# inferflow/inferflow

Measured on AMD Instinct MI355X. Metric: decode tokens/sec, Llama-2-7B Q4 batch=1 greedy (whole job), higher is better.
Workload: dtype i8 (Q8 activations x Q4_B32T1A weights, i32 dot, f32 scale, f16 I/O); 1 GPU; llama2_7b decode, Q4_B32T1A weights + F16 lm_head, F16 KV cache, batch 1 greedy, 16-token prompt, context 21..1851; parallelism=single, weights_bytes=4309647360

## Files before the change

include/inferflow_amd.h:

```cpp
#ifndef INFERFLOW_AMD_H_
#define INFERFLOW_AMD_H_

#include <stddef.h>
#include <stdint.h>

#ifdef __cplusplus
extern "C" {
#endif

typedef enum {
    IFA_F32 = 0, IFA_F16 = 1,
    IFA_Q8_B32T1 = 7, IFA_Q8_B32T2 = 8, IFA_Q6_B64T1 = 9, IFA_Q5_B64T1 = 10, IFA_Q5_B32T1 = 11,
    IFA_Q4_B16 = 12, IFA_Q4_B32T1A = 13, IFA_Q4_B32T1B = 14, IFA_Q4_B64T1 = 17, IFA_Q3H_B64T1 = 18,
    IFA_Q3_B32T1A = 19, IFA_Q3_B32T1B = 20, IFA_Q2_B32T1A = 21, IFA_Q2_B32T1B = 22
} ifa_dtype;

enum {
    IFA_OK = 0,
    IFA_ERR_ARG = -1,
    IFA_ERR_DTYPE = -2,
    IFA_ERR_HIP = -3,
    IFA_ERR_STATE = -4,
    IFA_ERR_NOMEM = -5
};
// ... 111 lines not shown
    IFA_T_EMBD = 0, IFA_T_OUT_NORM = 1, IFA_T_OUT_NORM_B = 2, IFA_T_LM_HEAD = 3,
    IFA_T_ATTN_NORM = 10, IFA_T_ATTN_NORM_B = 11, IFA_T_WQ = 12, IFA_T_WK = 13, IFA_T_WV = 14, IFA_T_WO = 15,
    IFA_T_FFN_NORM = 16, IFA_T_FFN_NORM_B = 17, IFA_T_W1 = 18, IFA_T_W2 = 19, IFA_T_W3 = 20, IFA_T_MOE_GATE = 21,
    IFA_T_WQ_B = 22, IFA_T_WK_B = 23, IFA_T_WV_B = 24, IFA_T_WO_B = 25, IFA_T_W1_B = 26, IFA_T_W2_B = 27, IFA_T_W3_B = 28,
    IFA_T_ATTN_POST_NORM = 29, IFA_T_ATTN_POST_NORM_B = 30, IFA_T_FFN_POST_NORM = 31, IFA_T_FFN_POST_NORM_B = 32
};

int ifa_model_create(const ifa_model_config *cfg, ifa_model **out);
int ifa_model_destroy(ifa_model *m);
int ifa_model_set_tensor(ifa_model *m, int layer, int tensor_id, int expert, int dtype,
                         const void *dev_src, size_t rows, size_t cols);
int ifa_model_set_tensor_f16(ifa_model *m, int layer, int tensor_id, int expert, int target_dtype,
                             const void *dev_src_f16, size_t rows, size_t cols);
int ifa_model_finalize(ifa_model *m);
int ifa_model_reset(ifa_model *m);
int ifa_model_kv_slots(ifa_model *m, int n_slots);
int ifa_model_select_kv(ifa_model *m, int slot);
int ifa_model_kv_copy(ifa_model *m, int src_slot, int dst_slot, int n_rows);
int ifa_model_set_option(ifa_model *m, const char *name, int value);
int ifa_model_set_excluded_tokens(ifa_model *m, const int *ids_host, int n);
int ifa_model_perf_stat(ifa_model *m, int *keys_out, float *ms_out, int cap, int *n_out, int clear);
int ifa_model_fused_supported(ifa_model *m, char *why, size_t why_len);
int ifa_model_forward(ifa_model *m, const int *tokens_host, int n_tokens, int prefix_len,
                      void *logits_out_dev, int *next_token_host);
int ifa_model_decode(ifa_model *m, int first_token, int start_pos, int n_steps,
                     int *out_tokens_host, float *elapsed_ms);
int ifa_model_decode_prepare(ifa_model *m, int start_pos, int n_steps);
int ifa_model_decode_batch(ifa_model *m, int n, const int *tokens_host, const int *positions_host, const int *kv_slots_host,
                           int *next_tokens_host, void *logits_out_dev);
int ifa_model_decode_draft(ifa_model *m, int n, const int *tokens_host, int pos0, int *next_tokens_host, void *logits_out_dev);
// ... 72 lines not shown
```

inferflow_amd/_capi.py:

```python
import ctypes as C
import os

_HERE = os.path.dirname(os.path.abspath(__file__))
_LIB_PATH = os.environ.get("IFA_LIB") or os.path.join(_HERE, "lib", "libinferflow_amd.so")
_lib = None


class IfaError(RuntimeError):
    def __init__(self, code, msg):
        super().__init__("inferflow_amd error %d: %s" % (code, msg))
        self.code = code


def library_path():
    return _LIB_PATH


def lib():
    global _lib
    if _lib is None:
        if not os.path.exists(_LIB_PATH):
            raise ImportError(
                "inferflow_amd: %s is missing -- run `python __graft_entry__.py build` "
                "(hipcc --offload-arch=gfx950); there is no CPU fallback" % _LIB_PATH)
# ... 81 lines not shown
    "ifa_add_by_row_index": (_i, [_vp, _vp, _sz, _sz, _vp, _vp, _vp]),
    "ifa_model_kv_slots": (_i, [_vp, _i]),
    "ifa_model_select_kv": (_i, [_vp, _i]),
    "ifa_model_kv_copy": (_i, [_vp, _i, _i, _i]),
    "ifa_model_decode_batch": (_i, [_vp, _i, _vp, _vp, _vp, _vp, _vp]),
    "ifa_model_decode_draft": (_i, [_vp, _i, _vp, _i, _vp, _vp]),
    "ifa_model_set_pool_excluded": (_i, [_vp, _vp, _i]),
    "ifa_model_decode_pool": (_i, [_vp, _i, _i, _i, _vp, _vp, _vp, _vp]),
    "ifa_model_decode_batch_pool": (_i, [_vp, _i, _vp, _vp, _vp, _vp, _i, _vp, _i, _vp, _vp, _vp]),
    "ifa_model_forward_pool": (_i, [_vp, _vp, _i, _i, _vp, _i, _vp, _vp, _vp, _vp]),
    "ifa_model_pool_lse": (_i, [_vp, _vp, _i, _vp]),
    "ifa_model_forward_score": (_i, [_vp, _vp, _i, _i, _vp, _vp, _vp, _vp]),
    "ifa_model_get_buffer": (_i, [_vp, C.c_char_p, _i, C.POINTER(_vp), C.POINTER(_sz)]),
    "ifa_model_stream": (_vp, [_vp]),
    "ifa_model_time_kernel": (_i, [_vp, _i, _i, _vp]),
    "ifa_model_set_stream": (_i, [_vp, _vp]),
    "ifa_model_tp_begin": (_i, [_vp, _i, _i]),
    "ifa_model_tp_begin_hidden": (_i, [_vp, _vp, _i]),
    "ifa_model_tp_hidden": (_i, [_vp, _vp]),
    "ifa_model_tp_attn": (_i, [_vp, _i, _vp]),
    "ifa_model_tp_post_attn": (_i, [_vp, _i, _vp]),
    "ifa_model_tp_ffn": (_i, [_vp, _i, _vp]),
    "ifa_model_tp_post_ffn": (_i, [_vp, _i, _vp]),
    "ifa_model_tp_logits": (_i, [_vp, _vp]),
    "ifa_model_tp_set_token": (_i, [_vp, _vp]),
    "ifa_comm_unique_id": (_i, [_vp]),
    "ifa_comm_init_rank": (_i, [_vp, _i, _i, _i, C.POINTER(_vp)]),
    "ifa_comm_init_all": (_i, [_vp, _i, C.POINTER(_vp)]),
    "ifa_comm_destroy": (_i, [_vp]),
    "ifa_comm_capturable": (_i, [_vp]),
# ... 93 lines not shown
```

inferflow_amd/csrc/ifa_decode_qkv_attn.h:

```cpp
#pragma once
#include "ifa_decode_kernels.h"
#include "ifa_decode_attn.h"

namespace ifa {

struct DecQkvAttnExtra {
    unsigned long long *gran;
    const unsigned *epoch;
    unsigned epoch_add;
    unsigned *err;
    int timeout_us;
    int gk;
    int unload;
};

#ifndef IFA_QA_EARLY_KV
#define IFA_QA_EARLY_KV 0
#endif
#ifndef IFA_QA_WARM_ROWS
#define IFA_QA_WARM_ROWS 1
#endif
constexpr int QA_THREADS = 512;

template <int DT, int NJ, int RW, int NORM, int HD, bool Q8, int PB, bool KT, int NP, bool UL = false>
__global__ void __launch_bounds__(QA_THREADS) k_dec_qkv_attn(const half_t *px, const half_t *pnw, const half_t *pnb, int pcols, int pgeo,
                                                             const uint8_t *pwq, const uint8_t *pwk, const uint8_t *pwv,
                                                             const DecGemvParams P, const DecAttnParams A, const DecQkvAttnExtra E)
{
    const int g_heads = pgeo & 0xFF, g_kvh = (pgeo >> 8) & 0xFF, g_gk = (pgeo >> 16) & 0xFFFF;
    const int g_nblk = pcols / block_capacity(DT);
    extern __shared__ __attribute__((aligned(16))) char smem[];
    const long long t_kernel = wall_clock64();
    static_assert(NORM == 0 || NORM == 1, "QKV prologue: quantiser with or without the RMS norm");
    static_assert(NP > 0 && NP * 64 < QA_THREADS, "wave-specialised prologue");
    constexpr int TH = QA_THREADS, PT = NP * 64;
    constexpr int MAXC = (NJ * 8 * block_capacity(DT) + PT - 1) / PT;
    XPre<NORM, MAXC, false, PT> pre;
    if (threadIdx.x < PT) pre.issue(px, pnw, pnb, pcols);
    const XLds L = xlds_carve(smem, pcols);
    const int lane = threadIdx.x & 63;
    const int wave = __builtin_amdgcn_readfirstlane(threadIdx.x >> 6);
    using Fmt = DecFmt<DT, NJ>;
    const size_t row_bytes = tiled_row_bytes(DT, (size_t)g_nblk);
    const int g = (int)blockIdx.x / g_gk, bg = (int)blockIdx.x - g * g_gk;
    const int group = g_heads / g_kvh;
    const int RG = (group + 2) * HD;
    const int per = g_gk / group;
    const bool attn_wg = bg % per == 0;
    const int head = g * group + bg / per;
    const int WGV = UL ? (g_gk - group) * (TH / 64) : g_gk * (TH / 64);
    const int lw = UL ? (bg - bg / per - 1) * (TH / 64) + wave : bg * (TH / 64) + wave;
    struct Row { const uint8_t *w; const half_t *b; half_t *y; int row, vrow; };
    auto locate = [&](int lr) {
        Row r;
        const int nq = group * HD;
        const bool isk = lr >= nq && lr < nq + HD, isv = lr >= nq + HD;
        r.row = isv ? g * HD + (lr - nq - HD) : (isk ? g * HD + (lr - nq) : g * nq + lr);
        r.w = isv ? P.W0[2] : (isk ? P.W0[1] : P.W0[0]);
        r.b = isv ? P.b0[2] : (isk ? P.b0[1] : P.b0[0]);
// ... 20 lines not shown
                if (i < i0 || i >= i1) continue;
                if (i > 0 && i * WGV + lw >= RG) continue;
                w[i].load(wrow(min(i * WGV + lw, RG - 1)), g_nblk, lane);
            }
        }
    };
    static_assert(NP == 4, "the prologue waves are the attention waves");
    const bool ul_head = UL && attn_wg;
    if (!ul_head && threadIdx.x == TH - 1) { L.part[130] = 0.0f; L.part[131] = 0.0f; }
    if (!ul_head && wave >= NP) load_rows(0, 1);
    const int pos = *(const __attribute__((address_space(4))) int *)(A.state + 1);
    const unsigned epoch = ((*(const __attribute__((address_space(4))) unsigned *)(E.epoch) + E.epoch_add) << 20) | ((unsigned)pos & 0xFFFFFu);
    DecAttnFusedIn F;
    F.gran = E.gran; F.epoch = epoch; F.pos = pos; F.err = E.err; F.timeout_ticks = (long long)E.timeout_us * 100;
    F.att_gran = nullptr;
    if constexpr (UL) {
        if (attn_wg) {
            if (wave >= 4) {
#if IFA_QA_WARM_ROWS
                if (pos >= PB) {
                    constexpr int SB = Q8 ? (HD / 32) * 34 : HD * 2;
                    const int kvh = head / group, kv_dim = g_kvh * HD;
                    const size_t rb = Q8 ? (size_t)(kv_dim / 32) * 34 : (size_t)kv_dim * 2;
                    const size_t ho = Q8 ? (size_t)((kvh * HD) / 32) * 34 : (size_t)kvh * HD * 2;
                    const int t = (int)threadIdx.x - 256;
                    const int off = min((t & 3) * 64, SB - 4) & ~1;
                    typedef uint32_t u32_a2 __attribute__((aligned(2)));
                    uint32_t acc = 0;
                    for (int j = PB + (t >> 2); j <= pos; j += 64) {
                        acc ^= *(const __attribute__((address_space(1))) u32_a2 *)(A.kcache + (size_t)j * rb + ho + off);
                        acc ^= *(const __attribute__((address_space(1))) u32_a2 *)(A.vcache + (size_t)j * rb + ho + off);
                    }
                    if (acc == 0x9E3779B9u && A.trace) A.trace[(size_t)A.heads * 8 + 7] = (long long)acc;
                }
#endif
                return;
            }
            DecAttnRegs<HD, Q8, PB, KT> RU;
            dec_attn_body<HD, Q8, false, PB, KT, true>(smem, nullptr, A.kcache, A.vcache, A.heads, A.kv_heads, A, head, F, RU);
            return;
        }
    }
    __syncthreads();
    DecAttnRegs<HD, Q8, PB, KT> R;
    if (wave >= NP) {
        load_rows(1, RW);
    } else {
        pre.finish(P.norm_w, P.norm_b, P.multi_base, P.eps, P.cols, L, P.xn_out, nullptr);
        load_rows(0, RW);
#if IFA_QA_EARLY_KV
        if (attn_wg) dec_attn_body<HD, Q8, false, PB, KT, true, 1>(smem, nullptr, A.kcache, A.vcache, A.heads, A.kv_heads, A, head, F, R);
#endif
    }
    lds_counter_wait(L.part + 131, NP);
    typename Fmt::X X;
    X.load(L.codes, L.scale, L.xsum, lane, g_nblk);
    {
        float a[RW];
#pragma unroll
        for (int i = 0; i < RW; i++) a[i] = w[i].dot(X);
#pragma unroll
        for (int i = 0; i < RW; i++) a[i] = wave_sum(a[i]);
        float a0 = 0.0f;
#pragma unroll
        for (int i = 0; i < RW; i++) { if (lane == i) a0 = a[i]; }
        const int lr = lane * WGV + lw;
        if (lane < RW && lr < RG) {
            const Row r = locate(lr);
            half_t y = dec_bias(a0, r.b, r.row);
            if (P.pre_scale != 0.0f) y = f2h(h2f(y) * P.pre_scale);
            r.y[r.row] = y;
            __hip_atomic_store(E.gran + r.vrow, ((unsigned long long)epoch << 32) | (unsigned long long)__builtin_bit_cast(uint16_t, y),
                               __ATOMIC_RELAXED, __HIP_MEMORY_SCOPE_AGENT);
        }
    }
    if (A.trace && threadIdx.x == 0) {
        A.trace[(size_t)(A.heads + (int)blockIdx.x) * 8 + 0] = t_kernel;
        A.trace[(size_t)(A.heads + (int)blockIdx.x) * 8 + 1] = wall_clock64();
    }
    if (attn_wg) {
        __syncthreads();
        if (wave >= 4) return;
        dec_attn_body<HD, Q8, false, PB, KT, true, IFA_QA_EARLY_KV ? 2 : 0>(smem, nullptr, A.kcache, A.vcache, A.heads, A.kv_heads, A, head, F, R);
        return;
    }
}

bool dec_qkv_attn_supported(int w_dtype, int cols, int heads, int kv_heads, int head_dim, int num_cus, int *gk_out, int *rw_out);
int dec_qkv_attn_launch(int w_dtype, int norm, bool kv_q8, int pb, bool kt, const DecGemvParams &P, const DecAttnParams &A, const DecQkvAttnExtra &E,
                        int max_ctx, hipStream_t s);
template <int DT>
int dec_qkv_attn_launch_dt(int norm, bool kv_q8, int pb, bool kt, int rw, const DecGemvParams &P, const DecAttnParams &A, const DecQkvAttnExtra &E,
                           int max_ctx, hipStream_t s);
// ... 3 lines not shown
```

inferflow_amd/csrc/ifa_dqkvattn_q4b32.hip:

```cpp
#include <algorithm>
#include "ifa_dqkvattn_impl.h"

namespace ifa {

extern template int dec_qkv_attn_launch_dt<Q3H_B64T1>(int, bool, int, bool, int, const DecGemvParams &, const DecAttnParams &, const DecQkvAttnExtra &, int, hipStream_t);
template int dec_qkv_attn_launch_dt<Q4_B32T1A>(int, bool, int, bool, int, const DecGemvParams &, const DecAttnParams &, const DecQkvAttnExtra &, int, hipStream_t);

bool dec_qkv_attn_supported(int w_dtype, int cols, int heads, int kv_heads, int head_dim, int num_cus, int *gk_out, int *rw_out)
{
    const bool q4 = w_dtype == Q4_B32T1A || w_dtype == Q4_B32T1B;
    if (!q4 && w_dtype != Q3H_B64T1) return false;
    if (head_dim != 128 || cols != 4096 || kv_heads < 1 || heads % kv_heads != 0) return false;
    if (num_cus < kv_heads || num_cus % kv_heads != 0) return false;
    const int gk = num_cus / kv_heads, group = heads / kv_heads;
    if (gk % group != 0) return false;
    const int rg = (group + 2) * head_dim, wv = gk * (QA_THREADS / 64);
    if (rg % wv != 0) return false;
    const int rw = rg / wv;
    if (rw != 6 && rw != 3) return false;
    if (gk_out) *gk_out = gk;
    if (rw_out) *rw_out = rw;
    return true;
}

// ... 3 lines not shown
    DecGemvParams P = P0;
    P.trace = nullptr;
    P.total_rows = P.rows[0] + P.rows[1] + P.rows[2];
    P.nblk = P.cols / block_capacity(w_dtype);
    int gk = 0, rw = 0;
    if (!dec_qkv_attn_supported(w_dtype, P.cols, A.heads, A.kv_heads, 128, A.kv_heads * E.gk, &gk, &rw) || gk != E.gk)
        return ifa_fail(IFA_ERR_ARG, "fused QKV + attention: unsupported shape");
    switch (w_dtype) {
    case Q4_B32T1A: case Q4_B32T1B: return dec_qkv_attn_launch_dt<Q4_B32T1A>(norm, kv_q8, pb, kt, rw, P, A, E, max_ctx, s);
    case Q3H_B64T1: return dec_qkv_attn_launch_dt<Q3H_B64T1>(norm, kv_q8, pb, kt, rw, P, A, E, max_ctx, s);
    default: return ifa_fail(IFA_ERR_DTYPE, "fused QKV + attention: dtype %d", w_dtype);
    }
}

}
```

inferflow_amd/csrc/ifa_engine.hip:

```cpp
#include "ifa_engine_state.h"

namespace ifae {

int perf_begin(ifa_model *m, int key)
{
    if (!m->opt_perf_stat) return -1;
    hipStreamCaptureStatus cs = hipStreamCaptureStatusNone;
    if (hipStreamIsCapturing(m->stream, &cs) != hipSuccess || cs != hipStreamCaptureStatusNone) { (void)hipGetLastError(); return -1; }
    auto take = [&]() -> hipEvent_t {
        if (!m->perf_pool.empty()) { hipEvent_t e = m->perf_pool.back(); m->perf_pool.pop_back(); return e; }
        hipEvent_t e = nullptr;
        if (hipEventCreate(&e) != hipSuccess) { (void)hipGetLastError(); return nullptr; }
        return e;
    };
    ifa_model::PerfSpanRec r; r.key = key; r.e0 = take(); r.e1 = take();
    if (!r.e0 || !r.e1) { if (r.e0) m->perf_pool.push_back(r.e0); if (r.e1) m->perf_pool.push_back(r.e1); return -1; }
    if (hipEventRecord(r.e0, m->stream) != hipSuccess) { (void)hipGetLastError(); m->perf_pool.push_back(r.e0); m->perf_pool.push_back(r.e1); return -1; }
    m->perf_spans.push_back(r);
    return (int)m->perf_spans.size() - 1;
}

void perf_end(ifa_model *m, int idx)
{
    if (idx < 0 || idx >= (int)m->perf_spans.size()) return;
// ... 6 lines not shown
    IFA_HIP_CHECK(hipStreamSynchronize(m->stream));
    for (auto &r : m->perf_spans) {
        float ms = 0.0f;
        if (hipEventElapsedTime(&ms, r.e0, r.e1) == hipSuccess) m->perf_map[r.key] += ms;
        else (void)hipGetLastError();
        m->perf_pool.push_back(r.e0); m->perf_pool.push_back(r.e1);
    }
    m->perf_spans.clear();
    return IFA_OK;
}

void drop_graphs(ifa_model *m)
{
    if (m->tp_graph_exec) { (void)hipGraphExecDestroy(m->tp_graph_exec); m->tp_graph_exec = nullptr; }
    if (m->tp_graph) { (void)hipGraphDestroy(m->tp_graph); m->tp_graph = nullptr; }
    if (m->graph_exec) { (void)hipGraphExecDestroy(m->graph_exec); m->graph_exec = nullptr; }
    if (m->graph) { (void)hipGraphDestroy(m->graph); m->graph = nullptr; }
    if (m->graph_exec_n) { (void)hipGraphExecDestroy(m->graph_exec_n); m->graph_exec_n = nullptr; }
    if (m->graph_n) { (void)hipGraphDestroy(m->graph_n); m->graph_n = nullptr; }
    for (auto &sl : m->slots) {
        if (sl.exec) { (void)hipGraphExecDestroy(sl.exec); sl.exec = nullptr; }
        if (sl.graph) { (void)hipGraphDestroy(sl.graph); sl.graph = nullptr; }
    }
    for (auto &kv : m->batch_graphs) if (kv.second) (void)hipGraphExecDestroy(kv.second);
    m->batch_graphs.clear();
    for (auto &kv : m->draft_graphs) if (kv.second) (void)hipGraphExecDestroy(kv.second);
    m->draft_graphs.clear();
}

void free_tensor(Tensor &t)
{
    if (t.data) (void)hipFree(t.data);
    if (t.tiled) (void)hipFree(t.tiled);
    if (t.mo) (void)hipFree(t.mo);
    if (t.x32) (void)hipFree(t.x32);
    if (t.q3hn) (void)hipFree(t.q3hn);
    t = Tensor();
}
// ... 430 lines not shown
    IFA_HIP_CHECK(hipStreamSynchronize(m->stream));
    return IFA_OK;
}

int ifa_model_select_kv(ifa_model *m, int slot)
{
    IFA_REQUIRE(m && m->finalized, "ifa_model_select_kv: model not finalized");
    if (m->slots.empty()) m->slots.resize(1);
    IFA_REQUIRE(slot >= 0 && slot < (int)m->slots.size(), "ifa_model_select_kv: slot %d of %zu", slot, m->slots.size());
    if (slot == m->cur_slot) return IFA_OK;
    if (m->tp_graph_exec) { (void)hipGraphExecDestroy(m->tp_graph_exec); m->tp_graph_exec = nullptr; }
    if (m->tp_graph) { (void)hipGraphDestroy(m->tp_graph); m->tp_graph = nullptr; }
    ifa_model::KvSlot &out = m->slots[(size_t)m->cur_slot], &in = m->slots[(size_t)slot];
    out.k.clear(); out.v.clear();
    for (Layer &L : m->layers) { out.k.push_back(L.kcache); out.v.push_back(L.vcache); }
    out.graph = m->graph; out.exec = m->graph_exec;
    if (m->graph_exec_n) { (void)hipGraphExecDestroy(m->graph_exec_n); m->graph_exec_n = nullptr; }
    if (m->graph_n) { (void)hipGraphDestroy(m->graph_n); m->graph_n = nullptr; }
    for (size_t l = 0; l < m->layers.size(); l++) { m->layers[l].kcache = in.k[l]; m->layers[l].vcache = in.v[l]; }
    m->graph = in.graph; m->graph_exec = in.exec;
    in.k.clear(); in.v.clear(); in.graph = nullptr; in.exec = nullptr;
    m->cur_slot = slot;
    return IFA_OK;
}

int ifa_model_set_option(ifa_model *m, const char *name, int value)
{
    IFA_REQUIRE(m && name, "ifa_model_set_option: null pointer");
    if (strcmp(name, "pool_lse") == 0) { m->opt_pool_lse = value != 0; return IFA_OK; }
    struct { const char *n; int *p; } opts[] = {
        {"fused", &m->opt_fused}, {"graph", &m->opt_graph}, {"rpw_qkv", &m->opt_rpw_qkv}, {"rpw_wo", &m->opt_rpw_wo},
        {"rpw_ffn", &m->opt_rpw_ffn}, {"rpw_w2", &m->opt_rpw_w2}, {"rpw_lm", &m->opt_rpw_lm}, {"trace", &m->opt_trace},
        {"bench_mode", &m->opt_bench_mode}, {"touch_stride", &m->opt_touch_stride}, {"attn_split_ctx", &m->opt_attn_split_ctx}, {"batch_graph", &m->opt_batch_graph}, {"gemm_rows", &m->opt_gemm_rows}, {"batch_fused", &m->opt_batch_fused}, {"rows_mo", &m->opt_rows_mo}, {"debug_mo_alloc_fail", &m->opt_debug_mo_alloc_fail}, {"rows_kparts", &m->opt_rows_kparts}, {"prefill_chunk", &m->opt_prefill_chunk}, {"prefill_big_min", &m->opt_prefill_big_min}, {"prefill_mid", &m->opt_prefill_mid}, {"prefill_mid_max", &m->opt_prefill_mid_max}, {"prefill_res_mid", &m->opt_prefill_res_mid}, {"gemm_splitk", &m->opt_gemm_splitk}, {"moe_singles", &m->opt_moe_singles}, {"moe_overlap", &m->opt_moe_overlap}, {"prefill_big", &m->opt_prefill_big}, {"moe_router_fused", &m->opt_moe_router_fused}, {"tp_fuse_add", &m->opt_tp_fuse_add}, {"attn_q8", &m->opt_attn_q8}, {"attn_kt", &m->opt_attn_kt}, {"fuse_attn", &m->opt_fuse_attn}, {"fuse_ffn", &m->opt_fuse_ffn}, {"attn_post_as_residual", &m->opt_attn_post_as_residual}, {"chain_late_w2", &m->opt_chain_late_w2}, {"exact_order", &m->opt_exact_order}, {"perf_stat", &m->opt_perf_stat}, {"attn_nsplits", &m->opt_attn_nsplits}, {"attn_unload", &m->opt_attn_unload}, {"q3h_native", &m->opt_q3h_native}, {"fuse_attn_timeout_us", &m->opt_fuse_attn_timeout_us}, {"step_tail", &m->opt_step_tail}, {"graph_steps", &m->opt_graph_steps}, {"moe_device", &m->opt_moe_device}, 
        
        {"debug_layers", &m->opt_debug_layers}, {"debug_layer0", &m->opt_debug_layer0}, {"debug_hidden_in", &m->opt_debug_hidden_in}};
    for (auto &o : opts)
        if (strcmp(o.n, name) == 0) {
            *o.p = value;
            drop_graphs(m);
            return IFA_OK;
        }
    return ifa_fail(IFA_ERR_ARG, "ifa_model_set_option: unknown option '%s'", name);
}

int ifa_model_perf_stat(ifa_model *m, int *keys_out, float *ms_out, int cap, int *n_out, int clear)
{
    IFA_REQUIRE(m && n_out && cap >= 0 && (cap == 0 || (keys_out && ms_out)), "ifa_model_perf_stat: null pointer");
    IFA_HIP_CHECK(hipSetDevice(m->cfg.device));
// ... 105 lines not shown
```

inferflow_amd/csrc/ifa_engine_decode.hip:

```cpp
#include "ifa_engine_state.h"

namespace ifae {

bool qkv_attn_layer_ok(const ifa_model *m, int l, int *gk_out);

static int attn_split_threshold(const ifa_model *m)
{
    if (m->opt_attn_split_ctx >= 0) return m->opt_attn_split_ctx;
    const ifa_model_config &c = m->cfg;
    bool tail = m->opt_attn_unload && m->opt_fuse_attn && waits_enabled() && dec_attn_smem(c.head_dim, c.max_ctx, 256) <= IFA_LDS_LIMIT;
    int gk = 0;
    for (int l = 0; tail && l < c.layers; l++) if (!qkv_attn_layer_ok(m, l, &gk)) tail = false;
    if (tail && (long long)c.kv_heads * gk > (long long)visible_cus()) tail = false;
    if (!tail) return 320;
    return c.heads > c.kv_heads ? 640 : 512;
}

void choose_attn_split(ifa_model *m, int reach)
{
    const int thr = attn_split_threshold(m);
    const int want = (thr > 0 && reach > thr) ? (reach > 8192 ? 16 : 8) : 0;
    if (want != m->attn_split) { m->attn_split = want; drop_graphs(m); }
    const int pb = reach <= 64 ? 64 : (reach <= 128 ? 128 : 256);
    if (pb != m->attn_pb) { m->attn_pb = pb; drop_graphs(m); }
}

__global__ void __launch_bounds__(256) k_touch(const uint8_t *__restrict__ p, size_t bytes, size_t stride, int *sink)
{
    size_t i = ((size_t)blockIdx.x * blockDim.x + threadIdx.x) * stride;
    int acc = 0;
    for (; i < bytes; i += (size_t)gridDim.x * blockDim.x * stride) acc += *reinterpret_cast<const int *>(p + i);
    if (acc == 0x7FFFFFFF) *sink = acc;
}

static long long *g_trace_ptr = nullptr;

bool fused_ok(const Tensor &t, bool long_rows)
{
    if (!t.present()) return false;
    if (fused_int8(t.dtype)) return t.tiled && (long_rows ? dec_gemv_supported_long(t.dtype, t.cols) : dec_gemv_supported(t.dtype, t.cols));
    return dec_gemv_h_supported(t.dtype, t.cols) && (long_rows || t.cols <= 8192);
}

template <int EPI, int NORM>
static int launch_dec_gemv(int w_dtype, const DecGemvParams &P, int wgs_per_cu_opt, hipStream_t s)
{
    if (!fused_int8(w_dtype) && w_dtype != Q3H_NATIVE) {
        if constexpr (NORM == 2 || epi_is_moe(EPI)) return ifa_fail(IFA_ERR_STATE, "fused GEMV: dtype %d has no kernel for this launch", w_dtype);
        else return dec_gemv_h_launch(w_dtype, EPI, NORM, P, s);
    }
    return dec_gemv_launch(w_dtype, EPI, NORM, P, wgs_per_cu_opt, s, g_trace_ptr);
}

int lmhead_grid(const DecLmHeadParams &P, int wgs_per_cu_opt)
{
    const int nj = (P.cols / 8 + 63) / 64;
    const int R = nj <= 4 ? 2 : 1;
    const int nbatch = (P.rows + R - 1) / R;
    const int per_cu = wgs_per_cu_opt > 0 ? wgs_per_cu_opt : 2;
    return std::max(1, std::min(num_cus() * per_cu, (nbatch + DEC_WAVES - 1) / DEC_WAVES));
}

int launch_lmhead(const DecLmHeadParams &P, int norm, int wgs_per_cu_opt, hipStream_t s, const DecStepTail *Z)
{
    const int chunks = P.cols / 8;
    const int nj = (chunks + 63) / 64;
// ... 162 lines not shown
    for (int i = 0; i < 3; i++) {
        P.W0[i] = wbytes(L.t[ids[i]]); P.b0[i] = (const half_t *)L.t[bids[i]].data;
        P.y[i] = outs[i]; P.rows[i] = (int)L.t[ids[i]].rows;
    }
    P.nsets = 3;
}

int launch_qkv_attn(ifa_model *m, int l, const half_t *x, unsigned tag_add)
{
    const ifa_model_config &c = m->cfg;
    Layer &L = m->layers[(size_t)l];
    DecGemvParams P; qkv_params(m, l, x, P);
    DecAttnParams A; attn_params(m, l, A);
    DecQkvAttnExtra E; memset(&E, 0, sizeof(E));
    E.gran = m->qa_gran + (size_t)l * (size_t)(c.heads + 2 * c.kv_heads) * c.head_dim;
    E.epoch = m->qa_call; E.epoch_add = tag_add; E.err = m->qa_err; E.timeout_us = m->opt_fuse_attn_timeout_us; E.gk = m->qa_gk;
    const int pb = (m->attn_pb == 64 || m->attn_pb == 128) ? m->attn_pb : 256;
    const bool kt = m->opt_attn_kt && !A.kv_q8 && dec_attn_smem(c.head_dim, c.max_ctx, pb) <= IFA_LDS_LIMIT;
    E.unload = ((m->opt_attn_unload >= 1 && pb == 256) || (m->opt_attn_unload >= 2 && pb == 128 && (kt || A.kv_q8))) ? 1 : 0;
    return dec_qkv_attn_launch(L.t[T_WQ].dtype, 1, A.kv_q8 != 0, pb, kt, P, A, E, c.max_ctx, m->stream);
}

int launch_qkv(ifa_model *m, int l, const half_t *x)
{
    const ifa_model_config &c = m->cfg;
    Layer &L = m->layers[(size_t)l];
    DecGemvParams P; memset(&P, 0, sizeof(P));
    P.x = x; P.norm_w = (const half_t *)L.t[T_ATTN_NORM].data; P.norm_b = (const half_t *)L.t[T_ATTN_NORM_B].data;
    P.multi_base = c.attn_norm_base; P.eps = c.eps; P.cols = c.dim; P.nblk = c.dim / 32;
    if (c.parallel_attn) P.xn_out = m->xn;
    const bool std_norm = c.norm_kind != 0;
// ... 254 lines not shown
    P.x = m->a; P.norm_w = (const half_t *)L.t[T_FFN_NORM].data; P.norm_b = (const half_t *)L.t[T_FFN_NORM_B].data;
    P.eps = c.eps; P.cols = c.dim; P.act_kind = c.act_kind; P.multi_base = c.ffn_norm_base;
    P.W0[0] = wbytes(L.t[T_W1]); P.b0[0] = (const half_t *)L.t[T_W1_B].data; P.y[0] = m->t1; P.rows[0] = (int)L.t[T_W1].rows;
    P.W1 = wbytes(L.t[T_W3]); P.b1 = (const half_t *)L.t[T_W3_B].data;
    DecGemvParams Q; memset(&Q, 0, sizeof(Q));
    Q.x = m->t1; Q.cols = (int)L.t[T_W2].cols; Q.eps = c.eps;
    Q.W0[0] = wbytes(L.t[T_W2]); Q.rows[0] = (int)L.t[T_W2].rows; Q.b0[0] = (const half_t *)L.t[T_W2_B].data;
    Q.y[0] = xnext; Q.residual = m->a;
    if (scale_on(c.ffn_out_scale)) Q.pre_scale = c.ffn_out_scale;
    if (l + 1 == c.layers && scale_on(c.out_scale)) Q.post_scale = c.out_scale;
    DecChainExtra E; memset(&E, 0, sizeof(E));
    const size_t per = (size_t)c.dim + L.t[T_W1].rows;
    E.gran_a = m->ch_gran + (size_t)l * per; E.gran_h = E.gran_a + c.dim;
    E.flags_a = m->ch_flags + (size_t)l * 2048; E.flags_h = E.flags_a + 1024;
    E.state = m->state; E.epoch = m->qa_call; E.epoch_add = tag_add; E.err = m->qa_err; E.timeout_us = m->opt_fuse_attn_timeout_us;
    E.trace = g_trace_ptr; E.late_w2 = m->opt_chain_late_w2;
    return dec_chain_launch(L.t[T_W1].dtype, true, 1, wo, P, Q, wo ? &PW : nullptr, E, num_cus(), m->stream);
}

bool step_tail_ok(const ifa_model *m)
{
    const ifa_model_config &c = m->cfg;
    return m->opt_step_tail && m->g[T_LM_HEAD].present() && m->g[T_LM_HEAD].dtype == F16 && m->g[T_EMBD].present()
        && !(c.norm_kind != 0 && m->g[T_OUT_NORM].present()) && c.dim % 8 == 0 && c.dim <= 8192;
}

DecLmHeadParams lm_params(ifa_model *m, const half_t *x, half_t *logits_out)
{
    const ifa_model_config &c = m->cfg;
    DecLmHeadParams H; memset(&H, 0, sizeof(H));
    H.x = x; H.norm_w = (const half_t *)m->g[T_OUT_NORM].data; H.norm_b = (const half_t *)m->g[T_OUT_NORM_B].data;
// ... 173 lines not shown
    };
    int rc = ensure_scratch(m, 1);
    if (rc) return rc;
    if (m->opt_q3h_native && (rc = ensure_q3hn(m))) return rc;
    hipStream_t s = m->stream;
    choose_attn_split(m, start_pos + n_steps);
    if ((rc = qkv_attn_ready(m))) return rc;
    if ((rc = step_tail_ready(m))) return rc;
    m->host_pinned[0] = first_token; m->host_pinned[1] = start_pos; m->host_pinned[2] = 0;
    IFA_HIP_CHECK(hipMemcpyAsync(m->state, m->host_pinned, 3 * sizeof(int), hipMemcpyHostToDevice, s));
    if (m->qa_on || m->ch_on) {
        m->qa_calls = (m->qa_calls % 4000u) + 1u;
        m->host_pinned[6] = (int)m->qa_calls;
        IFA_HIP_CHECK(hipMemcpyAsync(m->qa_call, m->host_pinned + 6, sizeof(int), hipMemcpyHostToDevice, s));
    }
    if (m->opt_graph && !m->graph_exec) {
        IFA_HIP_CHECK(hipStreamSynchronize(s));
        IFA_HIP_CHECK(hipStreamBeginCapture(s, hipStreamCaptureModeThreadLocal));
        rc = enqueue_fused_step(m);
        hipGraph_t gph = nullptr;
        hipError_t e = hipStreamEndCapture(s, &gph);
        if (rc) { if (gph) (void)hipGraphDestroy(gph); return rc; }
        if (e != hipSuccess) return ifa_fail(IFA_ERR_HIP, "hipStreamEndCapture: %s", hipGetErrorString(e));
        if (m->graph) (void)hipGraphDestroy(m->graph);
        m->graph = gph;
        IFA_HIP_CHECK(hipGraphInstantiate(&m->graph_exec, m->graph, nullptr, nullptr, 0));
    }
    const int S = m->opt_graph_steps;
    if (m->opt_graph && S > 1 && n_steps >= S && (!m->graph_exec_n || m->graph_n_steps != S)) {
        if (m->graph_exec_n) { (void)hipGraphExecDestroy(m->graph_exec_n); m->graph_exec_n = nullptr; }
        if (m->graph_n) { (void)hipGraphDestroy(m->graph_n); m->graph_n = nullptr; }
        IFA_HIP_CHECK(hipStreamSynchronize(s));
        IFA_HIP_CHECK(hipStreamBeginCapture(s, hipStreamCaptureModeThreadLocal));
        for (int i = 0; i < S && !rc; i++) rc = enqueue_fused_step(m);
        hipGraph_t gph = nullptr;
        hipError_t e = hipStreamEndCapture(s, &gph);
        if (rc) { if (gph) (void)hipGraphDestroy(gph); return rc; }
        if (e != hipSuccess) return ifa_fail(IFA_ERR_HIP, "hipStreamEndCapture: %s", hipGetErrorString(e));
        m->graph_n = gph; m->graph_n_steps = S;
        IFA_HIP_CHECK(hipGraphInstantiate(&m->graph_exec_n, m->graph_n, nullptr, nullptr, 0));
    }
    if (prepare_only) return IFA_OK;
    th("state copies enqueued");
    hipEvent_t e0 = nullptr, e1 = nullptr;
    if (elapsed_ms) { IFA_HIP_CHECK(hipEventCreate(&e0)); IFA_HIP_CHECK(hipEventCreate(&e1)); IFA_HIP_CHECK(hipEventRecord(e0, s)); }
    th("events created, first recorded");
    if (m->st_on && (rc = launch_gather(m))) return rc;
    for (int i = 0; i < n_steps;) {
        if (m->opt_graph && m->graph_exec_n && m->graph_n_steps == S && S > 1 && n_steps - i >= S) { IFA_HIP_CHECK(hipGraphLaunch(m->graph_exec_n, s)); i += S; continue; }
        if (m->opt_graph) IFA_HIP_CHECK(hipGraphLaunch(m->graph_exec, s));
        else if ((rc = enqueue_fused_step(m))) return rc;
        i++;
    }
    th("steps enqueued");
    if (elapsed_ms) IFA_HIP_CHECK(hipEventRecord(e1, s));
    if ((rc = pool_enqueue(m, m->logits, 1))) return rc;
    IFA_HIP_CHECK(hipMemcpyAsync(m->host_pinned + 8, m->state + 8, sizeof(int) * (size_t)n_steps, hipMemcpyDeviceToHost, s));
    int *qerr = m->host_pinned + 8 + ifa_model::RING;
    qerr[0] = 0;
    if (m->qa_on || m->ch_on) IFA_HIP_CHECK(hipMemcpyAsync(qerr, m->qa_err, 4, hipMemcpyDeviceToHost, s));
    th("copies back enqueued");
    IFA_HIP_CHECK(hipStreamSynchronize(s));
    th("stream synchronised");
    if (qerr[0] != 0) {
        (void)hipMemsetAsync(m->qa_err, 0, 16, s);
        (void)hipStreamSynchronize(s);
// ... 83 lines not shown
```

inferflow_amd/csrc/ifa_engine_state.h:

```cpp
#pragma once
#include <chrono>
#include <cstdlib>
#include <cstring>
#include <map>
#include <string>
#include <vector>
#include "ifa_host.h"
#include "ifa_decode_kernels.h"
#include "ifa_decode_attn.h"
#include "ifa_decode_gemv.h"
#include "ifa_moe.h"
#include "ifa_gemm_rows_mfma.h"
#include "ifa_gemm_big.h"
#include "ifa_decode_lmhead_tail.h"
#include "ifa_decode_singles.h"
#include "ifa_decode_qkv_attn.h"
#include "ifa_decode_chain.h"

using namespace ifa;

namespace ifae {


enum { T_EMBD = 0, T_OUT_NORM = 1, T_OUT_NORM_B = 2, T_LM_HEAD = 3,
// ... 48 lines not shown
    int *moe_route = nullptr;
    int *moe_idx = nullptr, *moe_pin = nullptr;
    int *moe_sel = nullptr, *moe_epos = nullptr, *moe_counts = nullptr;
    half_t *moe_selw = nullptr, *moe_g1 = nullptr, *moe_g3 = nullptr, *moe_gin = nullptr, *moe_gout = nullptr;
    uint8_t *moe_xq_in = nullptr, *moe_xq_mid = nullptr;
    void *moe_tiles = nullptr, *moe_singles = nullptr, *moe_smalls = nullptr;
    int opt_moe_device = 1;
    int *state = nullptr;
    float *rope_tab = nullptr;
    long long *trace = nullptr;
    int opt_trace = 0, opt_bench_mode = 0, opt_touch_stride = 65536;
    int *tokens_dev = nullptr;
    int *host_pinned = nullptr;
    int scratch_tokens = 0;
    size_t kv_row_bytes = 0;
    hipGraph_t graph = nullptr;
    hipGraphExec_t graph_exec = nullptr;
    hipGraph_t graph_n = nullptr; hipGraphExec_t graph_exec_n = nullptr; int graph_n_steps = 0, opt_graph_steps = 1;
    struct PendingAdd { const half_t *x = nullptr, *add = nullptr, *bias = nullptr; half_t *out = nullptr; bool on = false; } pend;
    int opt_tp_fuse_add = 1;
    void *batch_tab_dev = nullptr, *batch_tab_pin = nullptr;
    size_t batch_tab_bytes = 0;
    std::map<int, hipGraphExec_t> batch_graphs;
    std::map<int, hipGraphExec_t> draft_graphs;
    DecAttnSplitWs attn_ws = {nullptr, nullptr, nullptr, 8};
    int opt_attn_unload = 1;
    int opt_attn_nsplits = 0;
    int opt_fuse_attn = 1, opt_fuse_attn_timeout_us = 20000, qa_on = 0, qa_gk = 0;
    unsigned long long *qa_gran = nullptr;
    unsigned *qa_call = nullptr, *qa_err = nullptr, qa_calls = 0;
    int opt_fuse_ffn = 0, ch_on = 0, opt_chain_late_w2 = 0;
    int opt_q3h_native = 0;
    int opt_perf_stat = 0;
    struct PerfSpanRec { int key; hipEvent_t e0, e1; };
    std::vector<PerfSpanRec> perf_spans;
    std::vector<hipEvent_t> perf_pool;
    std::map<int, float> perf_map;
    int opt_exact_order = 0;
    float *exact_rope_tab = nullptr;
    uint32_t *ch_gran = nullptr, *ch_flags = nullptr;
    int opt_step_tail = 1, st_on = 0;
    unsigned long long *st_keys = nullptr; unsigned *st_counter = nullptr; int st_keys_n = 0;
    int attn_pb = 256, opt_attn_kt = 1;
    int attn_split = 0, opt_attn_split_ctx = -1, opt_batch_graph = 0, opt_gemm_rows = 1, opt_batch_fused = 1, opt_moe_router_fused = 1, opt_prefill_big = 1, opt_rows_mo = 1, opt_moe_singles = 1;
    struct KvSlot { std::vector<void *> k, v; hipGraph_t graph = nullptr; hipGraphExec_t exec = nullptr; };
    std::vector<KvSlot> slots;
    int cur_slot = 0;
    int opt_attn_q8 = 1;
    half_t *tp_a = nullptr, *tp_f = nullptr, *tp_hid = nullptr, *tp_logits = nullptr;
    float *tp_best = nullptr, *tp_gather = nullptr;
    int *tp_tok = nullptr;
    hipGraph_t tp_graph = nullptr;
    hipGraphExec_t tp_graph_exec = nullptr;
    struct TpKey {
        unsigned long long tp = 0, world = 0; int tp_size = 0, stage = 0, n_stages = 0, prev = 0, next = 0, src = 0, voff = 0, force = 0, fuse = 0, slot = 0, oneshot = 0;
        bool operator==(const TpKey &o) const { return tp == o.tp && world == o.world && tp_size == o.tp_size && stage == o.stage && n_stages == o.n_stages
                && prev == o.prev && next == o.next && src == o.src && voff == o.voff && force == o.force && fuse == o.fuse && slot == o.slot
                && oneshot == o.oneshot; }
    } tp_key;
    const ifa_tp_topology *topo = nullptr;
// ... 193 lines not shown
```

Measured before the change: 625.5 tokens/s.

## Select attention key-block bucket per decode step via per-bucket cached graphs

The step graph becomes a set of three captured graphs, one per attention key-block size (64/128/256). The decode loop picks the graph whose bucket matches each step's actual context length instead of using one bucket chosen for the whole call, so early steps of a call that crosses a bucket boundary can run smaller tiles. Changing the bucket no longer drops every graph, only the TP graph. The change also adds an XCD-aware block remap and a sibling KV warm-up prefetch, both disabled by default, plus tracing of the XCC id. The costs are extra graph captures and more code paths to maintain.

```diff
diff --git a/include/inferflow_amd.h b/include/inferflow_amd.h
--- a/include/inferflow_amd.h
+++ b/include/inferflow_amd.h
@@ -149,6 +149,7 @@
                              const void *dev_src_f16, size_t rows, size_t cols);
 int ifa_model_finalize(ifa_model *m);
 int ifa_model_reset(ifa_model *m);
+int ifa_dec_qkv_attn_block_map(int grid, int gk, int block);
 int ifa_model_kv_slots(ifa_model *m, int n_slots);
 int ifa_model_select_kv(ifa_model *m, int slot);
 int ifa_model_kv_copy(ifa_model *m, int src_slot, int dst_slot, int n_rows);
diff --git a/inferflow_amd/_capi.py b/inferflow_amd/_capi.py
--- a/inferflow_amd/_capi.py
+++ b/inferflow_amd/_capi.py
@@ -119,6 +119,7 @@
     "ifa_model_get_buffer": (_i, [_vp, C.c_char_p, _i, C.POINTER(_vp), C.POINTER(_sz)]),
     "ifa_model_stream": (_vp, [_vp]),
     "ifa_model_time_kernel": (_i, [_vp, _i, _i, _vp]),
+    "ifa_dec_qkv_attn_block_map": (_i, [_i, _i, _i]),
     "ifa_model_set_stream": (_i, [_vp, _vp]),
     "ifa_model_tp_begin": (_i, [_vp, _i, _i]),
     "ifa_model_tp_begin_hidden": (_i, [_vp, _vp, _i]),
diff --git a/inferflow_amd/csrc/ifa_decode_qkv_attn.h b/inferflow_amd/csrc/ifa_decode_qkv_attn.h
--- a/inferflow_amd/csrc/ifa_decode_qkv_attn.h
+++ b/inferflow_amd/csrc/ifa_decode_qkv_attn.h
@@ -12,7 +12,19 @@
     int timeout_us;
     int gk;
     int unload;
+    int warm;
 };
+
+#ifndef IFA_QA_XCD_MAP
+#define IFA_QA_XCD_MAP 0
+#endif
+__host__ __device__ inline int qa_block_map_xcd(int b, int grid, int gk)
+{
+    const int q = grid >> 3;
+    if ((grid & 7) != 0 || gk <= 0 || q % gk != 0) return b;
+    return (b & 7) * q + (b >> 3);
+}
+__host__ __device__ inline int qa_block_map(int b, int grid, int gk) { return IFA_QA_XCD_MAP ? qa_block_map_xcd(b, grid, gk) : b; }
 
 #ifndef IFA_QA_EARLY_KV
 #define IFA_QA_EARLY_KV 0
@@ -20,6 +32,10 @@
 #ifndef IFA_QA_WARM_ROWS
 #define IFA_QA_WARM_ROWS 1
 #endif
+#ifndef IFA_QA_SIBLING_WARM
+#define IFA_QA_SIBLING_WARM 0
+#endif
+constexpr int QA_GETREG_XCC_ID = 20 | (0 << 6) | ((4 - 1) << 11);
 constexpr int QA_THREADS = 512;
 
 template <int DT, int NJ, int RW, int NORM, int HD, bool Q8, int PB, bool KT, int NP, bool UL = false>
@@ -42,7 +58,8 @@
     const int wave = __builtin_amdgcn_readfirstlane(threadIdx.x >> 6);
     using Fmt = DecFmt<DT, NJ>;
     const size_t row_bytes = tiled_row_bytes(DT, (size_t)g_nblk);
-    const int g = (int)blockIdx.x / g_gk, bg = (int)blockIdx.x - g * g_gk;
+    const int vb = qa_block_map((int)blockIdx.x, g_kvh * g_gk, g_gk);
+    const int g = vb / g_gk, bg = vb - g * g_gk;
     const int group = g_heads / g_kvh;
     const int RG = (group + 2) * HD;
     const int per = g_gk / group;
@@ -93,8 +110,27 @@
     DecAttnFusedIn F;
     F.gran = E.gran; F.epoch = epoch; F.pos = pos; F.err = E.err; F.timeout_ticks = (long long)E.timeout_us * 100;
     F.att_gran = nullptr;
+    [[maybe_unused]] uint32_t warm_acc = 0;
+    [[maybe_unused]] auto sibling_warm = [&]() -> uint32_t {
+        constexpr int SB = Q8 ? (HD / 32) * 34 : HD * 2;
+        const int kv_dim = g_kvh * HD;
+        const size_t rb = Q8 ? (size_t)(kv_dim / 32) * 34 : (size_t)kv_dim * 2;
+        const size_t ho = Q8 ? (size_t)((g * HD) / 32) * 34 : (size_t)g * HD * 2;
+        const int t = ((bg - bg / per - 1) * (TH / 64 - NP) + (wave - NP)) * 64 + lane;
+        const int j = t >> 3;
+        const int off = min((t & 3) * 64, SB - 4) & ~1;
+        const bool on = E.warm != 0 && !attn_wg && j < pos;
+        const uint8_t *row = ((t & 4) ? A.vcache : A.kcache) + (size_t)max(j, 0) * rb + ho + off;
+        const uint8_t *p = on ? row : (const uint8_t *)A.state;
+        typedef uint32_t u32_a2 __attribute__((aligned(2)));
+        return *(const __attribute__((address_space(1))) u32_a2 *)p;
+    };
     if constexpr (UL) {
         if (attn_wg) {
+            if (A.trace && threadIdx.x == 0) {
+                A.trace[(size_t)(A.heads + (int)blockIdx.x) * 8 + 2] = (long long)(__builtin_amdgcn_s_getreg(QA_GETREG_XCC_ID) & 0xF);
+                A.trace[(size_t)(A.heads + (int)blockIdx.x) * 8 + 3] = ((long long)g << 16) | (long long)bg;
+            }
             if (wave >= 4) {
 #if IFA_QA_WARM_ROWS
                 if (pos >= PB) {
@@ -124,6 +160,9 @@
     DecAttnRegs<HD, Q8, PB, KT> R;
     if (wave >= NP) {
         load_rows(1, RW);
+#if IFA_QA_SIBLING_WARM
+        if constexpr (!UL) warm_acc = sibling_warm();
+#endif
     } else {
         pre.finish(P.norm_w, P.norm_b, P.multi_base, P.eps, P.cols, L, P.xn_out, nullptr);
         load_rows(0, RW);
@@ -153,9 +192,14 @@
                                __ATOMIC_RELAXED, __HIP_MEMORY_SCOPE_AGENT);
         }
     }
+#if IFA_QA_SIBLING_WARM
+    if (warm_acc == 0x9E3779B9u && A.trace) A.trace[(size_t)A.heads * 8 + 7] = (long long)warm_acc;
+#endif
     if (A.trace && threadIdx.x == 0) {
         A.trace[(size_t)(A.heads + (int)blockIdx.x) * 8 + 0] = t_kernel;
         A.trace[(size_t)(A.heads + (int)blockIdx.x) * 8 + 1] = wall_clock64();
+        A.trace[(size_t)(A.heads + (int)blockIdx.x) * 8 + 2] = (long long)(__builtin_amdgcn_s_getreg(QA_GETREG_XCC_ID) & 0xF);
+        A.trace[(size_t)(A.heads + (int)blockIdx.x) * 8 + 3] = ((long long)g << 16) | (long long)bg;
     }
     if (attn_wg) {
         __syncthreads();
diff --git a/inferflow_amd/csrc/ifa_dqkvattn_q4b32.hip b/inferflow_amd/csrc/ifa_dqkvattn_q4b32.hip
--- a/inferflow_amd/csrc/ifa_dqkvattn_q4b32.hip
+++ b/inferflow_amd/csrc/ifa_dqkvattn_q4b32.hip
@@ -41,3 +41,9 @@
 }
 
 }
+
+extern "C" int ifa_dec_qkv_attn_block_map(int grid, int gk, int block)
+{
+    if (gk < 1 || grid < 1 || grid % gk != 0 || block < 0 || block >= grid) return -1;
+    return ifa::qa_block_map_xcd(block, grid, gk);
+}
diff --git a/inferflow_amd/csrc/ifa_engine.hip b/inferflow_amd/csrc/ifa_engine.hip
--- a/inferflow_amd/csrc/ifa_engine.hip
+++ b/inferflow_amd/csrc/ifa_engine.hip
@@ -44,14 +44,16 @@
 {
     if (m->tp_graph_exec) { (void)hipGraphExecDestroy(m->tp_graph_exec); m->tp_graph_exec = nullptr; }
     if (m->tp_graph) { (void)hipGraphDestroy(m->tp_graph); m->tp_graph = nullptr; }
-    if (m->graph_exec) { (void)hipGraphExecDestroy(m->graph_exec); m->graph_exec = nullptr; }
-    if (m->graph) { (void)hipGraphDestroy(m->graph); m->graph = nullptr; }
+    auto drop_steps = [](ifa_model::StepGraphs &sg) {
+        for (int b = 0; b < 3; b++) {
+            if (sg.exec[b]) { (void)hipGraphExecDestroy(sg.exec[b]); sg.exec[b] = nullptr; }
+            if (sg.graph[b]) { (void)hipGraphDestroy(sg.graph[b]); sg.graph[b] = nullptr; }
+        }
+    };
+    drop_steps(m->sg);
     if (m->graph_exec_n) { (void)hipGraphExecDestroy(m->graph_exec_n); m->graph_exec_n = nullptr; }
     if (m->graph_n) { (void)hipGraphDestroy(m->graph_n); m->graph_n = nullptr; }
-    for (auto &sl : m->slots) {
-        if (sl.exec) { (void)hipGraphExecDestroy(sl.exec); sl.exec = nullptr; }
-        if (sl.graph) { (void)hipGraphDestroy(sl.graph); sl.graph = nullptr; }
-    }
+    for (auto &sl : m->slots) drop_steps(sl.sg);
     for (auto &kv : m->batch_graphs) if (kv.second) (void)hipGraphExecDestroy(kv.second);
     m->batch_graphs.clear();
     for (auto &kv : m->draft_graphs) if (kv.second) (void)hipGraphExecDestroy(kv.second);
@@ -512,12 +514,12 @@
     ifa_model::KvSlot &out = m->slots[(size_t)m->cur_slot], &in = m->slots[(size_t)slot];
     out.k.clear(); out.v.clear();
     for (Layer &L : m->layers) { out.k.push_back(L.kcache); out.v.push_back(L.vcache); }
-    out.graph = m->graph; out.exec = m->graph_exec;
+    out.sg = m->sg;
     if (m->graph_exec_n) { (void)hipGraphExecDestroy(m->graph_exec_n); m->graph_exec_n = nullptr; }
     if (m->graph_n) { (void)hipGraphDestroy(m->graph_n); m->graph_n = nullptr; }
     for (size_t l = 0; l < m->layers.size(); l++) { m->layers[l].kcache = in.k[l]; m->layers[l].vcache = in.v[l]; }
-    m->graph = in.graph; m->graph_exec = in.exec;
-    in.k.clear(); in.v.clear(); in.graph = nullptr; in.exec = nullptr;
+    m->sg = in.sg;
+    in.k.clear(); in.v.clear(); in.sg = ifa_model::StepGraphs();
     m->cur_slot = slot;
     return IFA_OK;
 }
@@ -529,7 +531,7 @@
     struct { const char *n; int *p; } opts[] = {
         {"fused", &m->opt_fused}, {"graph", &m->opt_graph}, {"rpw_qkv", &m->opt_rpw_qkv}, {"rpw_wo", &m->opt_rpw_wo},
         {"rpw_ffn", &m->opt_rpw_ffn}, {"rpw_w2", &m->opt_rpw_w2}, {"rpw_lm", &m->opt_rpw_lm}, {"trace", &m->opt_trace},
-        {"bench_mode", &m->opt_bench_mode}, {"touch_stride", &m->opt_touch_stride}, {"attn_split_ctx", &m->opt_attn_split_ctx}, {"batch_graph", &m->opt_batch_graph}, {"gemm_rows", &m->opt_gemm_rows}, {"batch_fused", &m->opt_batch_fused}, {"rows_mo", &m->opt_rows_mo}, {"debug_mo_alloc_fail", &m->opt_debug_mo_alloc_fail}, {"rows_kparts", &m->opt_rows_kparts}, {"prefill_chunk", &m->opt_prefill_chunk}, {"prefill_big_min", &m->opt_prefill_big_min}, {"prefill_mid", &m->opt_prefill_mid}, {"prefill_mid_max", &m->opt_prefill_mid_max}, {"prefill_res_mid", &m->opt_prefill_res_mid}, {"gemm_splitk", &m->opt_gemm_splitk}, {"moe_singles", &m->opt_moe_singles}, {"moe_overlap", &m->opt_moe_overlap}, {"prefill_big", &m->opt_prefill_big}, {"moe_router_fused", &m->opt_moe_router_fused}, {"tp_fuse_add", &m->opt_tp_fuse_add}, {"attn_q8", &m->opt_attn_q8}, {"attn_kt", &m->opt_attn_kt}, {"fuse_attn", &m->opt_fuse_attn}, {"fuse_ffn", &m->opt_fuse_ffn}, {"attn_post_as_residual", &m->opt_attn_post_as_residual}, {"chain_late_w2", &m->opt_chain_late_w2}, {"exact_order", &m->opt_exact_order}, {"perf_stat", &m->opt_perf_stat}, {"attn_nsplits", &m->opt_attn_nsplits}, {"attn_unload", &m->opt_attn_unload}, {"q3h_native", &m->opt_q3h_native}, {"fuse_attn_timeout_us", &m->opt_fuse_attn_timeout_us}, {"step_tail", &m->opt_step_tail}, {"graph_steps", &m->opt_graph_steps}, {"moe_device", &m->opt_moe_device}, 
+        {"bench_mode", &m->opt_bench_mode}, {"touch_stride", &m->opt_touch_stride}, {"attn_split_ctx", &m->opt_attn_split_ctx}, {"batch_graph", &m->opt_batch_graph}, {"gemm_rows", &m->opt_gemm_rows}, {"batch_fused", &m->opt_batch_fused}, {"rows_mo", &m->opt_rows_mo}, {"debug_mo_alloc_fail", &m->opt_debug_mo_alloc_fail}, {"rows_kparts", &m->opt_rows_kparts}, {"prefill_chunk", &m->opt_prefill_chunk}, {"prefill_big_min", &m->opt_prefill_big_min}, {"prefill_mid", &m->opt_prefill_mid}, {"prefill_mid_max", &m->opt_prefill_mid_max}, {"prefill_res_mid", &m->opt_prefill_res_mid}, {"gemm_splitk", &m->opt_gemm_splitk}, {"moe_singles", &m->opt_moe_singles}, {"moe_overlap", &m->opt_moe_overlap}, {"prefill_big", &m->opt_prefill_big}, {"moe_router_fused", &m->opt_moe_router_fused}, {"tp_fuse_add", &m->opt_tp_fuse_add}, {"attn_q8", &m->opt_attn_q8}, {"attn_kt", &m->opt_attn_kt}, {"fuse_attn", &m->opt_fuse_attn}, {"fuse_ffn", &m->opt_fuse_ffn}, {"attn_post_as_residual", &m->opt_attn_post_as_residual}, {"chain_late_w2", &m->opt_chain_late_w2}, {"exact_order", &m->opt_exact_order}, {"perf_stat", &m->opt_perf_stat}, {"attn_nsplits", &m->opt_attn_nsplits}, {"attn_unload", &m->opt_attn_unload}, {"q3h_native", &m->opt_q3h_native}, {"fuse_attn_timeout_us", &m->opt_fuse_attn_timeout_us}, {"step_tail", &m->opt_step_tail}, {"graph_steps", &m->opt_graph_steps}, {"moe_device", &m->opt_moe_device}, {"attn_pb_step", &m->opt_attn_pb_step}, {"attn_warm", &m->opt_attn_warm}, 
         
         {"debug_layers", &m->opt_debug_layers}, {"debug_layer0", &m->opt_debug_layer0}, {"debug_hidden_in", &m->opt_debug_hidden_in}};
     for (auto &o : opts)
diff --git a/inferflow_amd/csrc/ifa_engine_decode.hip b/inferflow_amd/csrc/ifa_engine_decode.hip
--- a/inferflow_amd/csrc/ifa_engine_decode.hip
+++ b/inferflow_amd/csrc/ifa_engine_decode.hip
@@ -16,13 +16,20 @@
     return c.heads > c.kv_heads ? 640 : 512;
 }
 
+static inline int attn_bucket(int keys) { return keys <= 64 ? 64 : (keys <= 128 ? 128 : 256); }
+static inline int attn_bucket_idx(int pb) { return pb == 64 ? 0 : (pb == 128 ? 1 : 2); }
+
 void choose_attn_split(ifa_model *m, int reach)
 {
     const int thr = attn_split_threshold(m);
     const int want = (thr > 0 && reach > thr) ? (reach > 8192 ? 16 : 8) : 0;
     if (want != m->attn_split) { m->attn_split = want; drop_graphs(m); }
-    const int pb = reach <= 64 ? 64 : (reach <= 128 ? 128 : 256);
-    if (pb != m->attn_pb) { m->attn_pb = pb; drop_graphs(m); }
+    const int pb = attn_bucket(reach);
+    if (pb != m->attn_pb) {
+        m->attn_pb = pb;
+        if (m->tp_graph_exec) { (void)hipGraphExecDestroy(m->tp_graph_exec); m->tp_graph_exec = nullptr; }
+        if (m->tp_graph) { (void)hipGraphDestroy(m->tp_graph); m->tp_graph = nullptr; }
+    }
 }
 
 __global__ void __launch_bounds__(256) k_touch(const uint8_t *__restrict__ p, size_t bytes, size_t stride, int *sink)
@@ -34,6 +41,7 @@
 }
 
 static long long *g_trace_ptr = nullptr;
+static bool g_trace_qa_only = false;
 
 bool fused_ok(const Tensor &t, bool long_rows)
 {
@@ -49,7 +57,7 @@
         if constexpr (NORM == 2 || epi_is_moe(EPI)) return ifa_fail(IFA_ERR_STATE, "fused GEMV: dtype %d has no kernel for this launch", w_dtype);
         else return dec_gemv_h_launch(w_dtype, EPI, NORM, P, s);
     }
-    return dec_gemv_launch(w_dtype, EPI, NORM, P, wgs_per_cu_opt, s, g_trace_ptr);
+    return dec_gemv_launch(w_dtype, EPI, NORM, P, wgs_per_cu_opt, s, g_trace_qa_only ? nullptr : g_trace_ptr);
 }
 
 int lmhead_grid(const DecLmHeadParams &P, int wgs_per_cu_opt)
@@ -242,7 +250,7 @@
     DecAttnParams A; attn_params(m, l, A);
     DecQkvAttnExtra E; memset(&E, 0, sizeof(E));
     E.gran = m->qa_gran + (size_t)l * (size_t)(c.heads + 2 * c.kv_heads) * c.head_dim;
-    E.epoch = m->qa_call; E.epoch_add = tag_add; E.err = m->qa_err; E.timeout_us = m->opt_fuse_attn_timeout_us; E.gk = m->qa_gk;
+    E.epoch = m->qa_call; E.epoch_add = tag_add; E.err = m->qa_err; E.timeout_us = m->opt_fuse_attn_timeout_us; E.gk = m->qa_gk; E.warm = m->opt_attn_warm ? 1 : 0;
     const int pb = (m->attn_pb == 64 || m->attn_pb == 128) ? m->attn_pb : 256;
     const bool kt = m->opt_attn_kt && !A.kv_q8 && dec_attn_smem(c.head_dim, c.max_ctx, pb) <= IFA_LDS_LIMIT;
     E.unload = ((m->opt_attn_unload >= 1 && pb == 256) || (m->opt_attn_unload >= 2 && pb == 128 && (kt || A.kv_q8))) ? 1 : 0;
@@ -527,7 +535,7 @@
     E.gran_a = m->ch_gran + (size_t)l * per; E.gran_h = E.gran_a + c.dim;
     E.flags_a = m->ch_flags + (size_t)l * 2048; E.flags_h = E.flags_a + 1024;
     E.state = m->state; E.epoch = m->qa_call; E.epoch_add = tag_add; E.err = m->qa_err; E.timeout_us = m->opt_fuse_attn_timeout_us;
-    E.trace = g_trace_ptr; E.late_w2 = m->opt_chain_late_w2;
+    E.trace = g_trace_qa_only ? nullptr : g_trace_ptr; E.late_w2 = m->opt_chain_late_w2;
     return dec_chain_launch(L.t[T_W1].dtype, true, 1, wo, P, Q, wo ? &PW : nullptr, E, num_cus(), m->stream);
 }
 
@@ -731,20 +739,35 @@
         m->host_pinned[6] = (int)m->qa_calls;
         IFA_HIP_CHECK(hipMemcpyAsync(m->qa_call, m->host_pinned + 6, sizeof(int), hipMemcpyHostToDevice, s));
     }
-    if (m->opt_graph && !m->graph_exec) {
-        IFA_HIP_CHECK(hipStreamSynchronize(s));
-        IFA_HIP_CHECK(hipStreamBeginCapture(s, hipStreamCaptureModeThreadLocal));
-        rc = enqueue_fused_step(m);
-        hipGraph_t gph = nullptr;
-        hipError_t e = hipStreamEndCapture(s, &gph);
-        if (rc) { if (gph) (void)hipGraphDestroy(gph); return rc; }
-        if (e != hipSuccess) return ifa_fail(IFA_ERR_HIP, "hipStreamEndCapture: %s", hipGetErrorString(e));
-        if (m->graph) (void)hipGraphDestroy(m->graph);
-        m->graph = gph;
-        IFA_HIP_CHECK(hipGraphInstantiate(&m->graph_exec, m->graph, nullptr, nullptr, 0));
+    struct TraceScope { ~TraceScope() { g_trace_ptr = nullptr; g_trace_qa_only = false; } } trace_scope;
+    if (m->opt_trace >= 2) {
+        if (!m->trace) { IFA_HIP_CHECK(hipMalloc((void **)&m->trace, sizeof(long long) * 2048 * 8)); IFA_HIP_CHECK(hipMemsetAsync(m->trace, 0, sizeof(long long) * 2048 * 8, s)); }
+        g_trace_ptr = m->trace; g_trace_qa_only = true;
     }
     const int S = m->opt_graph_steps;
-    if (m->opt_graph && S > 1 && n_steps >= S && (!m->graph_exec_n || m->graph_n_steps != S)) {
+    const bool multi = m->opt_graph && S > 1 && n_steps >= S;
+    const bool stepwise = m->opt_attn_pb_step && !m->attn_split && !multi;
+    const int call_pb = m->attn_pb;
+    auto step_pb = [&](int i) { return stepwise ? attn_bucket(start_pos + i + 1) : call_pb; };
+    if (m->opt_graph) {
+        const int b0 = attn_bucket_idx(step_pb(0)), b1 = attn_bucket_idx(step_pb(n_steps - 1));
+        for (int b = b0; b <= b1; b++) {
+            if (m->sg.exec[b]) continue;
+            m->attn_pb = b == 0 ? 64 : (b == 1 ? 128 : 256);
+            IFA_HIP_CHECK(hipStreamSynchronize(s));
+            IFA_HIP_CHECK(hipStreamBeginCapture(s, hipStreamCaptureModeThreadLocal));
+            rc = enqueue_fused_step(m);
+            hipGraph_t gph = nullptr;
+            hipError_t e = hipStreamEndCapture(s, &gph);
+            m->attn_pb = call_pb;
+            if (rc) { if (gph) (void)hipGraphDestroy(gph); return rc; }
+            if (e != hipSuccess) return ifa_fail(IFA_ERR_HIP, "hipStreamEndCapture: %s", hipGetErrorString(e));
+            if (m->sg.graph[b]) (void)hipGraphDestroy(m->sg.graph[b]);
+            m->sg.graph[b] = gph;
+            IFA_HIP_CHECK(hipGraphInstantiate(&m->sg.exec[b], m->sg.graph[b], nullptr, nullptr, 0));
+        }
+    }
+    if (multi && (!m->graph_exec_n || m->graph_n_steps != S || m->graph_n_pb != call_pb)) {
         if (m->graph_exec_n) { (void)hipGraphExecDestroy(m->graph_exec_n); m->graph_exec_n = nullptr; }
         if (m->graph_n) { (void)hipGraphDestroy(m->graph_n); m->graph_n = nullptr; }
         IFA_HIP_CHECK(hipStreamSynchronize(s));
@@ -754,7 +777,7 @@
         hipError_t e = hipStreamEndCapture(s, &gph);
         if (rc) { if (gph) (void)hipGraphDestroy(gph); return rc; }
         if (e != hipSuccess) return ifa_fail(IFA_ERR_HIP, "hipStreamEndCapture: %s", hipGetErrorString(e));
-        m->graph_n = gph; m->graph_n_steps = S;
+        m->graph_n = gph; m->graph_n_steps = S; m->graph_n_pb = call_pb;
         IFA_HIP_CHECK(hipGraphInstantiate(&m->graph_exec_n, m->graph_n, nullptr, nullptr, 0));
     }
     if (prepare_only) return IFA_OK;
@@ -764,9 +787,14 @@
     th("events created, first recorded");
     if (m->st_on && (rc = launch_gather(m))) return rc;
     for (int i = 0; i < n_steps;) {
-        if (m->opt_graph && m->graph_exec_n && m->graph_n_steps == S && S > 1 && n_steps - i >= S) { IFA_HIP_CHECK(hipGraphLaunch(m->graph_exec_n, s)); i += S; continue; }
-        if (m->opt_graph) IFA_HIP_CHECK(hipGraphLaunch(m->graph_exec, s));
-        else if ((rc = enqueue_fused_step(m))) return rc;
+        if (multi && n_steps - i >= S) { IFA_HIP_CHECK(hipGraphLaunch(m->graph_exec_n, s)); i += S; continue; }
+        if (m->opt_graph) IFA_HIP_CHECK(hipGraphLaunch(m->sg.exec[attn_bucket_idx(step_pb(i))], s));
+        else {
+            m->attn_pb = step_pb(i);
+            rc = enqueue_fused_step(m);
+            m->attn_pb = call_pb;
+            if (rc) return rc;
+        }
         i++;
     }
     th("steps enqueued");
diff --git a/inferflow_amd/csrc/ifa_engine_state.h b/inferflow_amd/csrc/ifa_engine_state.h
--- a/inferflow_amd/csrc/ifa_engine_state.h
+++ b/inferflow_amd/csrc/ifa_engine_state.h
@@ -86,9 +86,9 @@
     int *host_pinned = nullptr;
     int scratch_tokens = 0;
     size_t kv_row_bytes = 0;
-    hipGraph_t graph = nullptr;
-    hipGraphExec_t graph_exec = nullptr;
+    struct StepGraphs { hipGraph_t graph[3] = {nullptr, nullptr, nullptr}; hipGraphExec_t exec[3] = {nullptr, nullptr, nullptr}; } sg;
     hipGraph_t graph_n = nullptr; hipGraphExec_t graph_exec_n = nullptr; int graph_n_steps = 0, opt_graph_steps = 1;
+    int graph_n_pb = 0;
     struct PendingAdd { const half_t *x = nullptr, *add = nullptr, *bias = nullptr; half_t *out = nullptr; bool on = false; } pend;
     int opt_tp_fuse_add = 1;
     void *batch_tab_dev = nullptr, *batch_tab_pin = nullptr;
@@ -114,8 +114,10 @@
     int opt_step_tail = 1, st_on = 0;
     unsigned long long *st_keys = nullptr; unsigned *st_counter = nullptr; int st_keys_n = 0;
     int attn_pb = 256, opt_attn_kt = 1;
+    int opt_attn_pb_step = 1;
+    int opt_attn_warm = 0;
     int attn_split = 0, opt_attn_split_ctx = -1, opt_batch_graph = 0, opt_gemm_rows = 1, opt_batch_fused = 1, opt_moe_router_fused = 1, opt_prefill_big = 1, opt_rows_mo = 1, opt_moe_singles = 1;
-    struct KvSlot { std::vector<void *> k, v; hipGraph_t graph = nullptr; hipGraphExec_t exec = nullptr; };
+    struct KvSlot { std::vector<void *> k, v; StepGraphs sg; };
     std::vector<KvSlot> slots;
     int cur_slot = 0;
     int opt_attn_q8 = 1;
```

Result: no change. 622.5 tokens/s (-0.5%).
